# PacificBiosciences/ccs

Hardware: AMD Instinct MI355X
Metric: ZMWs/sec (HiFi reads/sec), 10-pass x 10 kb synthetic (higher is better)
Workload: dtype f32

## Files before the change

ccs_amd/csrc/ccsx_api.cpp:

```cpp
#include <hip/hip_runtime.h>

#include <algorithm>
#include <cmath>
#include <cstdio>
#include <cstdlib>
#include <cstring>
#include <mutex>
#include <string>
#include <vector>

#include "ccsx.h"
#include "ccsx_internal.h"
#include "ccsx_kernels.h"

#define HIPTRY(expr)                                                                                           \
    do {                                                                                                       \
        hipError_t e_ = (expr);                                                                                \
        if (e_ != hipSuccess) {                                                                                \
            ccsx_set_error(std::string(#expr) + ": " + hipGetErrorString(e_));                                 \
            return -2;                                                                                         \
        }                                                                                                      \
    } while (0)

#define CCSX_SLOTS 3
// ... 909 lines not shown
}
int ccsx_polish_batch(ccsx_handle h, const ccsx_batch *b, const ccsx_drafts *drafts, ccsx_results *res, uint32_t flags)
{
    ccsx_ticket t;
    if (int rc = ccsx_submit_polish(h, b, drafts, res, flags, &t)) return rc;
    return ccsx_wait(h, t);
}

static Slot *slot_of(ccsx_handle h, ccsx_ticket t)
{
    if (!h || t < 0) return nullptr;
    Slot &S = h->slot[t % CCSX_SLOTS];
    return S.ticket == t ? &S : nullptr;
}

int ccsx_wait(ccsx_handle h, ccsx_ticket ticket)
{
    Slot *S = slot_of(h, ticket);
    if (!S) { ccsx_set_error("ccsx_wait: unknown or recycled ticket"); return -1; }
    HIPTRY(hipSetDevice(h->device));
    return retire(h, *S);
}

int ccsx_poll(ccsx_handle h, ccsx_ticket ticket)
{
    Slot *S = slot_of(h, ticket);
    if (!S) { ccsx_set_error("ccsx_poll: unknown or recycled ticket"); return -1; }
    const hipError_t e = hipEventQuery(S->ev_done);
    if (e == hipErrorNotReady) return 0;
    if (e != hipSuccess) { ccsx_set_error(std::string("ccsx_poll: ") + hipGetErrorString(e)); return -2; }
    HIPTRY(hipSetDevice(h->device));
    return retire(h, *S) ? -2 : 1;
}

int ccsx_ticket_timings(ccsx_handle h, ccsx_ticket ticket, ccsx_timings *t)
{
    Slot *S = slot_of(h, ticket);
    if (!S || !t || !(S->ran || S->tm_ok)) { ccsx_set_error("ccsx_ticket_timings: unknown ticket"); return -1; }
    if (S->tm_ok) { *t = S->tm; return 0; }
    HIPTRY(hipSetDevice(h->device));
    return slot_timings(h, *S, t);
}

static int upload_impl(ccsx_handle h, const ccsx_batch *b, bool pile, bool tandem = false, int min_tandem = 0)
{
    if (!h) { ccsx_set_error("ccsx_upload: null handle"); return -1; }
    HIPTRY(hipSetDevice(h->device));
    for (auto &S : h->slot) if (int rc = retire(h, S)) return rc;
    Slot &S = h->slot[0];
    S.ticket = -1;
    const int rc = stage(h, S, b, h->s_comp, pile, tandem, min_tandem);
    if (rc) { S.staged = false; return rc; }
    S.mode = CCSX_RUN_FUSED;
    HIPTRY(hipStreamSynchronize(h->s_comp));
    h->last = 0;
    return 0;
}

int ccsx_upload(ccsx_handle h, const ccsx_batch *b) { return upload_impl(h, b, false); }

int ccsx_run(ccsx_handle h)
{
    if (!h || !h->slot[0].staged || h->slot[0].mode != CCSX_RUN_FUSED) { ccsx_set_error("ccsx_run: no batch uploaded for the fused path: call ccsx_upload first"); return -1; }
    HIPTRY(hipSetDevice(h->device));
    h->last = 0;
    return launch(h, h->slot[0]);
}

int ccsx_sync(ccsx_handle h)
{
    if (!h) return -1;
    HIPTRY(hipSetDevice(h->device));
    HIPTRY(hipStreamSynchronize(h->s_draft));
    HIPTRY(hipStreamSynchronize(h->s_comp));
    Slot &S = h->slot[h->last];
#ifdef CCSX_PROFILE_PHASES
    if (S.staged && S.ran) {
        unsigned long long ph[16];
        HIPTRY(hipMemcpy(ph, S.P.phase, sizeof(ph), hipMemcpyDeviceToHost));
        static const char *nm[8] = {"prologue", "tables+lanes", "chunk plan", "fill", "score", "select/apply", "qv+store", "validity+list"};
        unsigned long long tot = 0;
        for (int i = 0; i < 8; ++i) tot += ph[i];
        for (int i = 0; i < 8; ++i) std::fprintf(stderr, "[ccsx phase] %-14s %6.2f %%  (%llu cycles)\n", nm[i], tot ? 100.0 * ph[i] / tot : 0.0, ph[i]);
        static const char *pn[6] = {"thr setup+read", "thr traceback", "thr ids+zero", "thr records", "thr order", "thr col records"};
        unsigned long long pt = 0;
        for (int i = 8; i < 14; ++i) pt += ph[i];
        for (int i = 8; i < 14; ++i) std::fprintf(stderr, "[ccsx phase] %-14s %6.2f %%  (%llu cycles)\n", pn[i - 8], pt ? 100.0 * ph[i] / pt : 0.0, ph[i]);
    }
#endif
#ifdef CCSX_DEBUG_CHECKS
    if (S.staged) {
        int32_t dbg[2] = {0, 0};
        HIPTRY(hipMemcpy(dbg, S.P.debug, 8, hipMemcpyDeviceToHost));
        if (dbg[0]) { ccsx_set_error("device bounds check failed: code " + std::to_string(dbg[0]) + " at kernel line " + std::to_string(dbg[1])); return -3; }
    }
#endif
    (void)S;
    return 0;
}

int ccsx_download(ccsx_handle h, ccsx_results *res)
{
    if (!h || !h->slot[0].ran || h->slot[0].mode != CCSX_RUN_FUSED || !res) { ccsx_set_error("ccsx_download: nothing to download: ccsx_upload + ccsx_run first"); return -1; }
    Slot &S = h->slot[0];
    if (int rc = check_results(S, res, S.P.out_kin != nullptr)) return rc;
    HIPTRY(hipSetDevice(h->device));
    if (int rc = enqueue_download(S, res, h->s_comp)) return rc;
    HIPTRY(hipStreamSynchronize(h->s_comp));
    finish_outputs(S, res, nullptr);
    return 0;
}

int ccsx_consensus_batch(ccsx_handle h, const ccsx_batch *b, ccsx_results *res)
{
    int rc;
    if ((rc = ccsx_upload(h, b))) return rc;
    if ((rc = ccsx_run(h))) return rc;
    if ((rc = ccsx_sync(h))) return rc;
    return ccsx_download(h, res);
}

int ccsx_pileup_rule_version(void) { return 1; }

int ccsx_consensus_pileup(ccsx_handle h, const ccsx_batch *b, ccsx_results *res, ccsx_pileup *pile)
{
    if (!h || !b || !res || !pile) { ccsx_set_error("ccsx_consensus_pileup: null argument"); return -1; }
    int rc;
    if ((rc = upload_impl(h, b, true))) return rc;
    Slot &S = h->slot[0];
    if ((rc = check_pile(S, pile))) return rc;
    if ((rc = ccsx_run(h)) || (rc = ccsx_sync(h)) || (rc = ccsx_download(h, res))) return rc;
    if ((rc = enqueue_pile_download(S, pile, h->s_comp))) return rc;
    HIPTRY(hipStreamSynchronize(h->s_comp));
    return 0;
}

int ccsx_tandem_rule_version(void) { return 1; }

int ccsx_consensus_extras(ccsx_handle h, const ccsx_batch *b, ccsx_results *res, const ccsx_extras *ex)
{
    if (!h || !b || !res) { ccsx_set_error("ccsx_consensus_extras: null argument"); return -1; }
    bool tandem = false;
    if (extras_want(ex, &tandem)) return -1;
    ccsx_pileup *pile = ex ? ex->pile : nullptr;
    int rc;
    if ((rc = upload_impl(h, b, pile != nullptr, tandem, tandem ? ex->min_tandem_repeat_length : 0))) return rc;
    Slot &S = h->slot[0];
    if (pile && (rc = check_pile(S, pile))) return rc;
    if ((rc = ccsx_run(h)) || (rc = ccsx_sync(h)) || (rc = ccsx_download(h, res))) return rc;
    if (pile && (rc = enqueue_pile_download(S, pile, h->s_comp))) return rc;
    if (tandem && ex->tandem_len) HIPTRY(hipMemcpyAsync(ex->tandem_len, S.P.tlen, (size_t)S.P.n_zmw * 4, hipMemcpyDeviceToHost, h->s_comp));
    HIPTRY(hipStreamSynchronize(h->s_comp));
    return 0;
}

int ccsx_consensus_hd(ccsx_handle h, const ccsx_batch *b, ccsx_results *res, const ccsx_extras *ex, const ccsx_hd_request *hd)
{
    ccsx_hd_opts hdo{};
    if (b && hd_request_check(hd, b, &hdo, "ccsx_consensus_hd")) return -1;
    if (!h || !b || !res || !hd) { ccsx_set_error("ccsx_consensus_hd: null argument"); return -1; }
    bool tandem = false;
    if (extras_want(ex, &tandem)) return -1;
    ccsx_pileup *pile = ex ? ex->pile : nullptr;
    int rc;
    if ((rc = upload_impl(h, b, pile != nullptr, tandem, tandem ? ex->min_tandem_repeat_length : 0))) return rc;
    Slot &S = h->slot[0];
    if (pile && (rc = check_pile(S, pile))) return rc;
    if ((rc = check_results(S, res, S.P.out_kin != nullptr))) return rc;
    if ((rc = hd_table(h)) || (rc = hd_attach(h, S, hdo, hd->split, h->s_comp))) return rc;
    HIPTRY(hipStreamSynchronize(h->s_comp));
// ... 228 lines not shown
```

ccs_amd/csrc/ccsx_kernels.hip:

```cpp
#include <hip/hip_runtime.h>
#include <stdint.h>
#include <cstdio>
#include <cstdlib>

#include "ccsx.h"
#include "ccsx_kernels.h"
#include "wave_ops.h"

#define LANDED(x) asm volatile("" : "+v"(x))

#if (defined(CCSX_EXP_NO_FILL) || defined(CCSX_EXP_NO_SCORE) || defined(CCSX_EXP_ONE_ROUND) || defined(CCSX_EXP_ALL_VALID) || defined(CCSX_EXP_CHEAP_VALIDITY) || \
     defined(CCSX_EXP_NO_ROWS) || defined(CCSX_EXP_NO_SCORE_LOG) || defined(CCSX_EXP_SKIP_ROUND2_SCORE) || defined(CCSX_EXP_NO_QV_EXP) || defined(CCSX_EXP_REPEAT) || defined(CCSX_EXP_NO_BANDMASK) || \
     defined(CCSX_EXP_HOT_PROLOGUE) || defined(CCSX_EXIT_AFTER_PROLOGUE)) && !defined(CCSX_EXPERIMENT)
#error "CCSX_EXP_* / CCSX_EXIT_AFTER_PROLOGUE switches produce wrong results: build them with -DCCSX_EXPERIMENT (never ship such a library)"
#endif
#define CCSX_STR2(x) #x
#define CCSX_STR(x) CCSX_STR2(x)
int ccsx_kernel_is_experiment()
{
#ifdef CCSX_EXPERIMENT
    return 1;
#else
    return 0;
#endif
// ... 669 lines not shown
        }
        if (multim) {
            const int np = (rec.x >> 8) & 15;
            const bool act = live && k < n0;
            for (int q = 1; q < CCSX_MAXPRED; ++q) {
                if ((actm & M_SGT(np, q)) == 0ull) break;
                const bool on = act && np > q;
                int pq = q == 1 ? rec.z : rec.w, plo = q == 1 ? plo1 : plo2;
                if (q >= 3) {
                    if (on) {
                        pq = pxw[(size_t)k * 4 + (q - 3)];
                        if (k - pq > PRING) plo = kinfo[pq].x; else plo = LDS_I32(kinBase + (uint32_t)(pq & (PRING - 1)) * 16);
                    }
                    LANDED(pq); LANDED(plo);
                }
                const bool farq = on && k - pq > PRING;
                const int off = r0w - plo;
                const int w = imed3(off + 3, 1, PGS - 3);
                const uint32_t src = ringBase + (on ? (uint32_t)(pq & (PRING - 1)) : (uint32_t)PRING) * (PGS * 4) + ((uint32_t)w << 2);
                int x0 = LDS_I32(src), y0 = LDS_I32(src + 4), y1 = LDS_I32(src + 8);
                if (__builtin_expect(M_NE0(farq ? 1 : 0) != 0ull, 0)) {
                    if (farq) {
                        const int32_t *Mu = Mcol + (size_t)pq * PB;
                        const int o = off - 1;
                        x0 = (unsigned)o < (unsigned)PB ? Mu[o] : NEGV;
                        y0 = (unsigned)(o + 1) < (unsigned)PB ? Mu[o + 1] : NEGV;
                        y1 = (unsigned)(o + 2) < (unsigned)PB ? Mu[o + 2] : NEGV;
                    }
                    LANDED(x0); LANDED(y0); LANDED(y1);
                }
                const int mq = q << 1;
                int c;
                c = x0 + s0;     if (on && c > b0) { b0 = c; m0 = mq; }
                c = y0 + SC_DEL; if (on && c > b0) { b0 = c; m0 = mq | 1; }
                c = y0 + s1;     if (on && c > b1) { b1 = c; m1 = mq; }
                c = y1 + SC_DEL; if (on && c > b1) { b1 = c; m1 = mq | 1; }
            }
        }
        { const int c = b0 + SC_INS; if (c > b1) { b1 = c; m1 = 15; } }
        {
            const int S = row_scan_max_i32(b1 + l8);
            const int Sp = __builtin_amdgcn_update_dpp(-(1 << 30), S, DPP_ROW_SHR(1), 0xf, 0xf, false);
            const int c0v = Sp - (l8 - 8 - SC_INS);
            const int c1v = Sp - (l8 - 8 - 2 * SC_INS);
            if (c0v > b0) { b0 = c0v; m0 = 15; }
            if (c1v > b1) { b1 = c1v; m1 = 15; }
        }
        if (r0w > I || b0 < NEGV / 2) b0 = NEGV;
        if (r0w >= I || b1 < NEGV / 2) b1 = NEGV;
        int cm, br;
        {
            const int f = -(1 << 24);
            const int k0_ = ((b0 > f ? b0 : f) * 64) | kRow0, k1_ = ((b1 > f ? b1 : f) * 64) | kRow1;
            const int key = row_allmax_i32(k0_ > k1_ ? k0_ : k1_);
            cm = key >> 6; br = (lo + 63) - (key & 63);
        }
        if (__builtin_expect((actm & M_SGT(lo + PB, I)) != 0ull, 0)) {
            const int e = r0w == I ? b0 : (r0w + 1 == I ? b1 : NEGV);
            const int ev = __builtin_amdgcn_ds_bpermute(bcastAddr, row_scan_max_i32(e));
            if (live && k < n0 && ev > NEGV / 2 && ev > bs) { bs = ev; kend = k; }
        }
        if (live && k < n0) {
            *(int2 *)&sRing[gq][k & (PRING - 1)][4 + l2] = make_int2(b0, b1);
            *mvp = (uint8_t)(m0 | (m1 << 4));
            if (l == 0) {
                sKin[gq][k & (PRING - 1)] = make_int4(lo, cm, br, 0);
                *lop = lo;
            }
            if (__builtin_expect((rec.x & CREC_NEED) != 0, 0)) {
                *(int2 *)Mp = make_int2(b0, b1);
                if (l == 0) *kip = make_int4(lo, cm, br, p0);
            }
        }
    }
#undef M_NE0
#undef M_SLT
#undef M_SGT
#undef M_UGT
#undef LDS_I32
    __threadfence_block();
    if (live && l == 0) { st[ST_KEND] = kend; st[ST_BS] = bs; }
}

__global__ __launch_bounds__(64) __attribute__((amdgpu_waves_per_eu(8, 8))) void k_poa_thread(KParams P, int z0, int pass, int rr, int b0)
{
    const int bx = (int)blockIdx.x + b0;
    __shared__ __attribute__((aligned(16))) uint8_t sMv[TB_BLOCK * POA_MV_BYTES];
    const int lane = threadIdx.x;
    uint32_t *sread = dyn_lds;
    PoaSlot g = poa_slot(P, bx);
    if (z0 + bx >= P.n_zmw) return;
    if (!g.st[ST_LIVE] || !g.st[ST_OK] || rr >= g.st[ST_NPOA]) return;
    TPH_T0();
    const int z = rfl(P.zmw_perm[z0 + bx]);
    const int r0 = rfl(P.read_off[z]);
    const int bb = rfl(g.st[ST_BB]), nreads = rfl(g.st[ST_NREADS]), npoa = rfl(g.st[ST_NPOA]);
    const int r = r0 + (bb + rr < nreads ? bb + rr : bb + rr - nreads);
    const uint8_t *rb = P.bases + P.base_off[r];
    const int I = rfl((int)(P.base_off[r + 1] - P.base_off[r]));
    const int kend = rfl(g.st[ST_KEND]), bsc = rfl(g.st[ST_BS]);
    if (kend < 0 || bsc < I) return;
    const int rev = rfl(((P.flags[r] & 1) != g.st[ST_REV0]) ? 1 : 0);
    const int vcap = rfl(P.vcap[z]);
    const int n0 = rfl(g.st[ST_N]);
    const int par = rfl(g.st[ST_PAR]);
    const int4 *crec = par ? g.crec1 : g.crec0, *pxc = par ? g.px1 : g.px0;
    int4 *crec_nx = par ? g.crec0 : g.crec1, *px_nx = par ? g.px0 : g.px1;
    load_read_packed(sread, rb, I, rev, lane);
    __syncthreads();
    TPH(8);
    {
        int k = kend, i = I;
        int4 kiN = make_int4(0, 0, 0, -1), crN = make_int4(0, -1, -1, -1);
        int kbN = -1;
        uint4 mvN0 = make_uint4(0, 0, 0, 0);
        auto fetch = [&](int kb_) {
            const int kk = kb_ + lane;
            kbN = kb_;
            kiN = make_int4(0, 0, 0, -1); crN = make_int4(0, -1, -1, -1);
            if (kb_ >= 0) {
                if (kk < n0) { crN = crec[kk]; kiN = make_int4(g.loK[kk], 0, 0, crN.y); }
                mvN0 = ((const uint4 *)(g.mvK + (size_t)kb_ * POA_MV_BYTES))[lane];
            }
        };
        fetch((k / TB_BLOCK) * TB_BLOCK);
        while (k >= 0) {
            const int kb = (k / TB_BLOCK) * TB_BLOCK;
            if (kbN != kb) fetch(kb);
            __syncthreads();
            const int4 kiL = kiN, crL = crN;
            const int metaL = crN.x;
            ((uint4 *)sMv)[lane] = mvN0;
            fetch(kb - TB_BLOCK);
            __syncthreads();
            while (k >= kb) {
                int kl = k - kb;
                int mknown;
                {
                    const int kls = kl - lane;
                    const int src = kls & 63;
                    const int lo_s = __shfl(kiL.x, src), pp_s = __shfl(kiL.w, src);
                    const int off = i - lane - lo_s;
                    const bool inb = kls >= 0 && i - lane >= 1 && (unsigned)off < (unsigned)PB;
                    const int m_s = inb ? ((sMv[kls * POA_MV_BYTES + (off >> 1)] >> ((off & 1) << 2)) & 15) : 255;
                    const unsigned long long simple = __ballot(m_s == 0 && pp_s == k - lane - 1);
                    const int R = (simple == ~0ull) ? 64 : __ffsll((long long)~simple) - 1;
                    if (R > 0) {
                        const int meta_s = __shfl(metaL, src);
                        if (lane < R) {
                            const int ir = i - lane - 1;
                            g.pathv[ir] = ((meta_s & 3) == read_base_packed(sread, ir)) ? k - lane : -1;
                        }
                        k -= R; i -= R;
                        if (R >= 64 || k < kb) continue;
                        kl = k - kb;
                    }
                    mknown = rl(m_s, R);
                }
                const int lo_k = rl(kiL.x, kl);
                CHK(i - lo_k >= 0 && i - lo_k < PB && i >= 0, 101);
                const int mo = i - lo_k;
                const int m = mknown != 255 ? mknown : rfl((sMv[kl * POA_MV_BYTES + (mo >> 1)] >> ((mo & 1) << 2)) & 15);
                const int t = m == 15 ? MV_INS : (m & 1), slot = m >> 1;
                CHK(i >= 1 || t == MV_DEL, 102);
                if (t == MV_INS) { if (lane == 0) g.pathv[i - 1] = -1; --i; continue; }
                const int meta = rl(metaL, kl);
                const int np = (meta >> 8) & 15;
                int up;
                if (np == 0) up = -1;
                else if (slot == 0) up = rl(kiL.w, kl);
                else if (slot == 1) up = rl(crL.z, kl);
                else if (slot == 2) up = rl(crL.w, kl);
                else up = rfl(((const int32_t *)pxc)[(size_t)k * 4 + (slot - 3)]);
                if (t == MV_DIAG) {
                    if (lane == 0) g.pathv[i - 1] = ((meta & 3) == read_base_packed(sread, i - 1)) ? k : -1;
                    --i;
                }
                CHK(up < k && up >= -1, 103);
                k = up;
            }
            k = rfl(k); i = rfl(i);
        }
        for (int q = lane; q < i; q += LANES) g.pathv[q] = -1;
    }
    __threadfence_block();
    TPH(9);
    int32_t *cnt = g.bestK;
    auto newpos = [&](int q) -> int { return q + cnt[q]; };
    for (int q = lane; q <= n0; q += LANES) { cnt[q] = 0; g.onpK[q] = 0; }
    __threadfence_block();
    TPH(10);
    int lastEx = -1, nnew = 0;
    for (int c0 = 0; c0 < I; c0 += 2 * LANES) {
        int w[2], wn[2], ex[2];
        bool valid[2], isnew[2], lastOfRun[2];
#pragma unroll
        for (int u = 0; u < 2; ++u) {
            const int i = c0 + u * LANES + lane;
            valid[u] = i < I;
            const int ic = valid[u] ? i : I - 1;
            w[u] = g.pathv[ic];
            wn[u] = g.pathv[ic + 1 < I ? ic + 1 : ic];
        }
#pragma unroll
        for (int u = 0; u < 2; ++u) {
            const int i = c0 + u * LANES + lane;
            isnew[u] = valid[u] && w[u] < 0;
            nnew += __popcll(__ballot(isnew[u]));
            const int incl = wave_scan_max_i32((valid[u] && !isnew[u]) ? i : -1);
            int e = wave_shr1_i32(incl, -1);
            e = e > lastEx ? e : lastEx;
            ex[u] = e;
            const int li = rl(incl, 63);
            lastEx = li > lastEx ? li : lastEx;
            lastOfRun[u] = isnew[u] && ((i + 1 >= I) || (wn[u] >= 0));
        }
        int av[2];
#pragma unroll
        for (int u = 0; u < 2; ++u) av[u] = g.pathv[(lastOfRun[u] && ex[u] >= 0) ? ex[u] : 0];
#pragma unroll
        for (int u = 0; u < 2; ++u) {
            const int i = c0 + u * LANES + lane;
            if (valid[u] && !isnew[u]) g.onpK[w[u]] = 1;
            if (lastOfRun[u]) {
                const int ap = ex[u] >= 0 ? av[u] : -1;
                CHK(ap >= -1 && ap < n0, 106);
                cnt[ap + 1] = i - ex[u];
            }
        }
    }
    nnew = rfl(nnew);
    if (n0 + nnew > vcap) { if (lane == 0) g.st[ST_OK] = 0; return; }
    __threadfence_block();
    TPH(11);
    int carry = 0;
    for (int c0 = 0; c0 <= n0; c0 += 4 * LANES) {
        int cv[4];
#pragma unroll
        for (int u = 0; u < 4; ++u) { const int q = c0 + u * LANES + lane; cv[u] = cnt[q <= n0 ? q : n0]; }
#pragma unroll
        for (int u = 0; u < 4; ++u) {
            const int q = c0 + u * LANES + lane;
            const int incl = wave_scan_add_i32(q <= n0 ? cv[u] : 0);
            if (q <= n0) cnt[q] = carry + incl;
            carry += rl(incl, 63);
        }
    }
    const int n = n0 + nnew;
    for (int q = lane; q < n; q += LANES) g.needK[q] = 0;
    __threadfence_block();
    auto carry_over = [&](int q, int kn, int4 rec, int4 &pxr) -> int4 {
        const int np = (rec.x >> 8) & 15;
        rec.x &= ~CREC_FAR0;
        if (np > 0) { rec.y = newpos(rec.y); if (kn - rec.y > PRING) { g.needK[rec.y] = 1; rec.x |= CREC_FAR0; } }
        if (np > 1) { rec.z = newpos(rec.z); if (kn - rec.z > PRING) g.needK[rec.z] = 1; }
        if (np > 2) { rec.w = newpos(rec.w); if (kn - rec.w > PRING) g.needK[rec.w] = 1; }
        if (np > 3) {
            pxr = pxc[q];
            for (int e = 3; e < np; ++e) { const int pn = newpos(int4_get(pxr, e - 3)); int4_set(pxr, e - 3, pn); if (kn - pn > PRING) g.needK[pn] = 1; }
        }
        return rec;
    };
    for (int q0 = 0; q0 < n0; q0 += 2 * LANES) {
        int4 rec[2]; int kn[2]; bool go[2];
#pragma unroll
        for (int u = 0; u < 2; ++u) {
            const int q = q0 + u * LANES + lane;
            go[u] = q < n0 && !g.onpK[q < n0 ? q : 0];
            rec[u] = make_int4(0, -1, -1, -1); kn[u] = 0;
            if (go[u]) { rec[u] = crec[q]; kn[u] = newpos(q); }
        }
#pragma unroll
        for (int u = 0; u < 2; ++u) if (go[u]) {
            const int q = q0 + u * LANES + lane;
            int4 pxr = make_int4(-1, -1, -1, -1);
            const int4 r = carry_over(q, kn[u], rec[u], pxr);
            CHK(kn[u] >= 0 && kn[u] < n, 105);
            crec_nx[kn[u]] = r;
            if (((r.x >> 8) & 15) > 3) px_nx[kn[u]] = pxr;
        }
    }
    TPH(12);
    lastEx = -1;
    int prevP = -1;
    for (int c0 = 0; c0 < I; c0 += LANES) {
        const int i = c0 + lane;
        const bool valid = i < I;
        const int w = g.pathv[valid ? i : I - 1];
        const bool isnew = valid && w < 0;
        const int incl = wave_scan_max_i32((valid && !isnew) ? i : -1);
        int ex = wave_shr1_i32(incl, -1);
        ex = ex > lastEx ? ex : lastEx;
        { const int li = rl(incl, 63); lastEx = li > lastEx ? li : lastEx; }
        const int av = g.pathv[(isnew && ex >= 0) ? ex : 0];
        int4 rec = make_int4(0, -1, -1, -1);
        if (valid && !isnew) rec = crec[w];
        const int qa = valid ? (isnew ? (ex >= 0 ? av : 0) : w) : 0;
        int P = newpos(qa);
        if (isnew) P = (ex >= 0 ? P + 1 : 0) + (i - ex - 1);
        if (!valid) P = -1;
        int Pp = wave_shr1_i32(P, prevP);
        prevP = rl(P, 63);
        if (valid) {
            CHK(P >= 0 && P < n, 104);
            int4 pxr = make_int4(-1, -1, -1, -1);
            bool pxdirty = false;
            if (isnew) rec = make_int4(read_base_packed(sread, i) | ((Pp >= 0 ? 1 : 0) << 8) | (1 << CREC_NREADS_SHIFT), Pp, -1, -1);
            else {
                rec = carry_over(w, P, rec, pxr);
                rec.x += 1 << CREC_NREADS_SHIFT;
                if (Pp >= 0) {
                    const int np = (rec.x >> 8) & 15;
                    bool found = false;
                    if (np > 0) found |= rec.y == Pp;
                    if (np > 1) found |= rec.z == Pp;
                    if (np > 2) found |= rec.w == Pp;
                    for (int e = 3; e < np; ++e) found |= int4_get(pxr, e - 3) == Pp;
                    if (!found && np < CCSX_MAXPRED) {
                        if (np == 0) rec.y = Pp; else if (np == 1) rec.z = Pp; else if (np == 2) rec.w = Pp; else { int4_set(pxr, np - 3, Pp); pxdirty = true; }
                        rec.x += 1 << 8;
                        if (P - Pp > PRING) { g.needK[Pp] = 1; if (np == 0) rec.x |= CREC_FAR0; }
                    }
                }
            }
            crec_nx[P] = rec;
            if (((rec.x >> 8) & 15) > 3 || pxdirty) px_nx[P] = pxr;
        }
    }
    __threadfence_block();
    if (lane == 0) { g.st[ST_N] = n; g.st[ST_NADDED] += 1; g.st[ST_PAR] ^= 1; }
    (void)npoa;
    TPH(13);
}

__global__ __launch_bounds__(64) __attribute__((amdgpu_waves_per_eu(8, 8))) void k_poa_finish(KParams P, int z0, int pass, int b0)
{
    const int bx = (int)blockIdx.x + b0;
    const int lane = threadIdx.x;
    PoaSlot g = poa_slot(P, bx);
    if (z0 + bx >= P.n_zmw) return;
    if (!g.st[ST_LIVE]) return;
    const int z = rfl(P.zmw_perm[z0 + bx]);
    const int ok = rfl(g.st[ST_OK]), n = rfl(g.st[ST_N]), nadded = rfl(g.st[ST_NADDED]);
    const int4 *crec = g.st[ST_PAR] ? g.crec1 : g.crec0;
    const int32_t *pxw = (const int32_t *)(g.st[ST_PAR] ? g.px1 : g.px0);
    int Ld = 0, nw = 0, stat = -1;
    if (ok && n > 0) {
        int kbest = -1, sb = NEGV, best_prev = 0;
        for (int kb = 0; kb < n; kb += LANES) {
            const int kkL = kb + lane;
            int4 cL = make_int4(0, -1, -1, -1);
            if (kkL < n) cL = crec[kkL];
            const int nblk = (n - kb) < LANES ? (n - kb) : LANES;
            const int npL = (cL.x >> 8) & 15;
            const int wL = kkL < n ? 2 * ((cL.x >> CREC_NREADS_SHIFT) & 127) - nadded : 0;
            const int Pw = wave_scan_add_i32(wL);
            const bool headL = kkL < n && (lane == 0 || npL != 1 || cL.y != kkL - 1);
            unsigned long long heads = __ballot(headL);
            const unsigned long long headmask = heads;
            int hb = 0, bpv = kkL - 1;
            while (heads) {
                const int j = (int)__ffsll((long long)heads) - 1;
                heads &= heads - 1;
                const int k = kb + j;
                const int np = rl(npL, j);
                int b = 0, p = -1;
                for (int q = 0; q < np; ++q) {
                    int pu;
                    if (q < 3) pu = q == 0 ? rl(cL.y, j) : (q == 1 ? rl(cL.z, j) : rl(cL.w, j));
                    else pu = rfl(pxw[(size_t)k * 4 + (q - 3)]);
                    CHK(pu >= 0 && pu < k, 108);
                    int bu;
                    if (pu >= kb) {
                        const int pj = pu - kb;
                        const int hd = 63 - __clzll((long long)(headmask & ((2ull << pj) - 1ull)));
                        bu = rl(hb, hd) + rl(Pw, pj) - rl(Pw, hd);
                    } else bu = pu == kb - 1 ? best_prev : rfl(g.bestK[pu]);
// ... 2689 lines not shown
            const int i = atomicAdd(&sV[5], 1);
            if (i < CAP) sBuf[i] = ((unsigned long long)end << 32) | ((unsigned long long)s << 24) | ((unsigned long long)dist << 16) | (unsigned long long)(end - start);
        });
        __syncthreads();
    }
    const int nk = min(sV[5], CAP), n_listed = min(n_hits, NH);
    for (int i = tid; i < nk; i += NT) {
        const unsigned long long key = sBuf[i];
        int rank = 0;
        for (int q = 0; q < nk && rank < NH; ++q) rank += sBuf[q] < key ? 1 : 0;
        if (rank < NH) {
            const int end = (int)(key >> 32);
            list[rank * 3] = end - (int)(key & 0xffffu); list[rank * 3 + 1] = end; list[rank * 3 + 2] = (int)((key >> 24) & 0xffu) | ((int)((key >> 16) & 0xffu) << 8);
        }
    }
    if (tid < NH && tid >= n_listed) { list[tid * 3] = 0; list[tid * 3 + 1] = 0; list[tid * 3 + 2] = 0; }
    int cov = 0;
    for (int w = tid; w < words; w += NT) cov += __popc(sUnion[w]);
    if (cov) atomicAdd(&sV[4], cov);
    {
        const int seg = (L + NT - 1) / NT, a = min(tid * seg, L), b = min(a + seg, L);
        int lead = -1, run = 0, inner = 0;
        for (int i = a; i < b; ++i) {
            if ((sUnion[i >> 5] >> (i & 31)) & 1u) { if (lead < 0) lead = run; inner = max(inner, run); run = 0; }
            else ++run;
        }
        sSeg[tid][0] = lead < 0 ? b - a : lead; sSeg[tid][1] = run; sSeg[tid][2] = lead < 0 ? -1 : inner;
    }
    __syncthreads();
    if (tid == 0) {
        int run = 0, gap = 0;
        for (int t = 0; t < NT; ++t) {
            if (sSeg[t][2] < 0) { run += sSeg[t][0]; continue; }
            gap = max(gap, max(run + sSeg[t][0], sSeg[t][2]));
            run = sSeg[t][1];
        }
        gap = max(gap, run);
        const ccsx_adapter_opts &o = P.adapt;
        const int first = n_hits ? sV[1] : -1, last = sV[2];
        int v = 0;
        if (n_hits >= o.min_copies && gap <= o.max_insert) v |= CCSX_ADAPTER_CONCAT;
        if (n_hits >= 1 && (first <= o.end_slack || last >= L - o.end_slack)) v |= CCSX_ADAPTER_NEAR_END;
        out[0] = 1; out[n] = v; out[2 * n] = n_hits; out[3 * n] = n_listed; out[4 * n] = sV[4]; out[5 * n] = gap; out[6 * n] = first; out[7 * n] = last;
        out[8 * n] = sV[3];
    }
}

#define LAUNCH_CHECK(name) do { if (hipGetLastError() != hipSuccess && !failed) failed = name; } while (0)
#define CALL_CHECK(fn, ...) do { if (fn(__VA_ARGS__) != hipSuccess && !failed) failed = #fn; } while (0)
const char *ccsx_launch_all(const KParams &P, hipStream_t st, hipStream_t st_polish, hipEvent_t *ev , int mode, hipStream_t st_aux, hipEvent_t *ev_aux )
{
    const char *failed = nullptr;
    if (ev) CALL_CHECK(hipEventRecord, ev[0], st);
    CALL_CHECK(hipMemsetAsync, P.ticket_poa, 0, 256, st);
    CALL_CHECK(hipMemsetAsync, P.avalid, 0, (size_t)(P.n_reads > 0 ? P.n_reads : 1), st);
    if (P.tflag) { CALL_CHECK(hipMemsetAsync, P.tflag, 0, (size_t)P.n_zmw * 4, st); CALL_CHECK(hipMemsetAsync, P.tlen, 0, (size_t)P.n_zmw * 4, st); }
    {
        int n = P.n_zmw * CCSX_NCTX;
        hipLaunchKernelGGL(k_setup, dim3((n + 255) / 256), dim3(256), 0, st, P);
        LAUNCH_CHECK("k_setup");
    }
    trace_sync(st, "k_setup");
    if (ev) CALL_CHECK(hipEventRecord, ev[1], st);
    const size_t lds_read = (((size_t)P.maxL_max + 15) / 16) * 4 + 64 + 4 * (CCSX_MAX_PASSES + 1);
    const bool caller_drafts = mode == CCSX_RUN_POLISH || mode == CCSX_RUN_HD;
    if (caller_drafts) {
        hipLaunchKernelGGL(k_draft_in, dim3(P.n_zmw), dim3(64), 0, st, P);
        LAUNCH_CHECK("k_draft_in");
    }
    for (int pass = 0; pass < ((P.opts.no_fallback_draft || caller_drafts) ? 1 : 3); ++pass) {
        int cov = pass ? 2 * P.opts.max_poa_cov : P.opts.max_poa_cov;
        if (cov > PW_MAXREADS_SPEC) cov = PW_MAXREADS_SPEC;
        if (cov > P.max_reads) cov = P.max_reads;
        for (int z0 = 0; z0 < P.n_zmw && !caller_drafts; z0 += P.poa_slots) {
            const int nb = (P.n_zmw - z0) < P.poa_slots ? (P.n_zmw - z0) : P.poa_slots;
            auto poa_range = [&](hipStream_t s, int g0, int ng, hipEvent_t after_first_dp, hipEvent_t before_first_dp) {
                hipLaunchKernelGGL(k_poa_init, dim3(ng), dim3(64), lds_read, s, P, z0, pass, g0);
                LAUNCH_CHECK("k_poa_init");
                if (before_first_dp) CALL_CHECK(hipStreamWaitEvent, s, before_first_dp, 0);
                for (int rr = 1; rr < cov && pass < 2; ++rr) {
                    hipLaunchKernelGGL(k_poa_dp, dim3((ng + 3) / 4), dim3(64), 0, s, P, z0, pass, rr, g0 / 4);
                    LAUNCH_CHECK("k_poa_dp");
                    if (rr == 1 && after_first_dp) CALL_CHECK(hipEventRecord, after_first_dp, s);
                    hipLaunchKernelGGL(k_poa_thread, dim3(ng), dim3(64), lds_read, s, P, z0, pass, rr, g0);
                    LAUNCH_CHECK("k_poa_thread");
                }
                if (pass < 2) {
                    hipLaunchKernelGGL(k_poa_finish, dim3(ng), dim3(64), 0, s, P, z0, pass, g0);
                    LAUNCH_CHECK("k_poa_finish");
                }
            };
            if (st_aux && ev_aux && pass == 0 && cov > 1 && nb >= 4096) {
                const int ha = ((nb / 2) + 3) & ~3;
                CALL_CHECK(hipEventRecord, ev_aux[0], st);
                CALL_CHECK(hipStreamWaitEvent, st_aux, ev_aux[0], 0);
                poa_range(st, 0, ha, ev_aux[1], nullptr);
                poa_range(st_aux, ha, nb - ha, nullptr, ev_aux[1]);
                CALL_CHECK(hipEventRecord, ev_aux[2], st_aux);
                CALL_CHECK(hipStreamWaitEvent, st, ev_aux[2], 0);
            } else poa_range(st, 0, nb, nullptr, nullptr);
        }
        trace_sync(st, "k_poa");
        if (P.tflag) {
            hipLaunchKernelGGL(k_sdust, dim3(P.n_zmw), dim3(64), (size_t)CCSX_SDUST_TABLE_BYTES + (size_t)P.sdust_words * 4, st, P, pass);
            LAUNCH_CHECK("k_sdust");
        }
        if (ev && pass == 0) CALL_CHECK(hipEventRecord, ev[2], st);
        CALL_CHECK(hipMemsetAsync, P.align_retry, 0, 64, st);
        bool tb_aside_out = false; int tb_launches = 0;
        {
            const size_t lds16 = 4 * (CH16 / 16 + 3) * sizeof(uint32_t);
            static const bool aside_ok = [] { const char *e = getenv("CCSX_TB_ASIDE"); return !(e && e[0] == '0'); }();
            const bool aside = aside_ok && st_aux && ev_aux && pass == 0 && P.n_quads >= 4096;
            bool tb_aside = false;
            int c = 0;
            for (int qb = 0; qb < P.n_quads; qb += P.align16_slots, ++c) {
                const int nb = (P.n_quads - qb) < P.align16_slots ? (P.n_quads - qb) : P.align16_slots;
                const int region = P.align16_regions > 1 ? (c & 1) : 0;
                if (aside && c >= 2) CALL_CHECK(hipStreamWaitEvent, st, ev_aux[5 + (c & 1)], 0);
                if (aside && c >= 1 && P.align16_regions <= 1) CALL_CHECK(hipStreamWaitEvent, st, ev_aux[5 + ((c - 1) & 1)], 0);
                hipLaunchKernelGGL(k_align16, dim3(nb), dim3(64), lds16, st, P, qb, pass, region);
                LAUNCH_CHECK("k_align16");
                hipStream_t s_tb = st;
                if (aside) {
                    CALL_CHECK(hipEventRecord, ev_aux[3 + (c & 1)], st);
                    CALL_CHECK(hipStreamWaitEvent, st_aux, ev_aux[3 + (c & 1)], 0);
                    s_tb = st_aux; tb_aside = true;
                }
                hipLaunchKernelGGL(k_align16_tb, dim3((4 * nb + 63) / 64), dim3(64), 0, s_tb, P, qb, nb, region);
                LAUNCH_CHECK("k_align16_tb");
                if (aside) CALL_CHECK(hipEventRecord, ev_aux[5 + (c & 1)], st_aux);
            }
            tb_launches = c;
            tb_aside_out = tb_aside;
        }
        {
            const int g = P.align_slots < 1 ? 1 : (P.align_slots > 4096 ? 4096 : P.align_slots);
            hipLaunchKernelGGL(k_align, dim3(g), dim3(64), lds_read, st, P, pass);
            LAUNCH_CHECK("k_align");
        }
        trace_sync(st, "k_align");
        if (P.align_slots >= 2) {
            const int g = P.align_slots / 2 > 2048 ? 2048 : P.align_slots / 2;
            hipLaunchKernelGGL(k_rescue, dim3(g), dim3(64), lds_read, st, P, pass);
            LAUNCH_CHECK("k_rescue");
        }
        if (tb_aside_out) for (int c = tb_launches > 2 ? tb_launches - 2 : 0; c < tb_launches; ++c)
            CALL_CHECK(hipStreamWaitEvent, st, ev_aux[5 + (c & 1)], 0);
        hipLaunchKernelGGL(k_post, dim3((P.n_zmw + 255) / 256), dim3(256), 0, st, P, pass);
        LAUNCH_CHECK("k_post");
    }
    if (mode == CCSX_RUN_DRAFT) {
        if (ev) for (int k : {3, 6, 4, 5}) CALL_CHECK(hipEventRecord, ev[k], st);
        return failed;
    }
    hipLaunchKernelGGL(k_wmap, dim3(1), dim3(1024), 0, st, P);
    LAUNCH_CHECK("k_wmap");
    hipLaunchKernelGGL(k_wmap_fill, dim3((P.n_zmw + 3) / 4), dim3(256), 0, st, P);
    LAUNCH_CHECK("k_wmap_fill");
    if (mode == CCSX_RUN_FUSED && P.fold_zi) {
        hipLaunchKernelGGL(k_fold, dim3(P.n_zmw), dim3(CCSX_FOLD_THREADS), (size_t)P.fold_bins * 4, st, P);
        LAUNCH_CHECK("k_fold");
        trace_sync(st, "k_fold");
    }
    if (mode == CCSX_RUN_FUSED && P.adapt_zi) {
        hipLaunchKernelGGL(k_adapter, dim3(P.n_zmw), dim3(CCSX_ADAPTER_THREADS), (size_t)P.adapt_words * 8, st, P);
// ... 68 lines not shown
```

Measured before the change: 38470.

## Split POA traceback into a separate kernel packing four ZMWs per wave

Moves the POA traceback out of k_poa_thread into a new k_poa_tb kernel. Each 64-lane wave runs four ZMWs in 16-lane groups, using wave-level barriers, prefetched global loads done with inline assembly, and ballot/bpermute run skipping. Read-base matching is deferred: pathv stores the node position tagged with the node's base, and consumers decode it with path_pos against the read base. The goal is to stop a single ZMW's serial traceback from holding a whole wave, at the cost of an extra kernel launch per read and a more complex path encoding.

```diff
diff --git a/ccs_amd/csrc/ccsx_api.cpp b/ccs_amd/csrc/ccsx_api.cpp
--- a/ccs_amd/csrc/ccsx_api.cpp
+++ b/ccs_amd/csrc/ccsx_api.cpp
@@ -1015,10 +1015,11 @@
         unsigned long long tot = 0;
         for (int i = 0; i < 8; ++i) tot += ph[i];
         for (int i = 0; i < 8; ++i) std::fprintf(stderr, "[ccsx phase] %-14s %6.2f %%  (%llu cycles)\n", nm[i], tot ? 100.0 * ph[i] / tot : 0.0, ph[i]);
-        static const char *pn[6] = {"thr setup+read", "thr traceback", "thr ids+zero", "thr records", "thr order", "thr col records"};
+        static const char *pn[6] = {"thr setup+read", "thr (unused)", "thr ids+zero", "thr records", "thr order", "thr col records"};
         unsigned long long pt = 0;
         for (int i = 8; i < 14; ++i) pt += ph[i];
         for (int i = 8; i < 14; ++i) std::fprintf(stderr, "[ccsx phase] %-14s %6.2f %%  (%llu cycles)\n", pn[i - 8], pt ? 100.0 * ph[i] / pt : 0.0, ph[i]);
+        std::fprintf(stderr, "[ccsx phase] %-14s %llu cycles\n[ccsx phase] %-14s %llu cycles  (k_poa_thread, all phases: %llu)\n", "tb setup", ph[14], "tb walk", ph[15], pt);
     }
 #endif
 #ifdef CCSX_DEBUG_CHECKS
diff --git a/ccs_amd/csrc/ccsx_kernels.hip b/ccs_amd/csrc/ccsx_kernels.hip
--- a/ccs_amd/csrc/ccsx_kernels.hip
+++ b/ccs_amd/csrc/ccsx_kernels.hip
@@ -775,10 +775,121 @@
     if (live && l == 0) { st[ST_KEND] = kend; st[ST_BS] = bs; }
 }
 
+#define TB_PATH_BASE_SHIFT 28
+#define TB_PATH_POS ((1 << TB_PATH_BASE_SHIFT) - 1)
+__device__ __forceinline__ int path_pos(int w, int read_base) { return (w >= 0 && (w >> TB_PATH_BASE_SHIFT) == read_base) ? (w & TB_PATH_POS) : -1; }
+
+__global__ __launch_bounds__(64) void k_poa_tb(KParams P, int z0, int pass, int rr, int b0)
+{
+    const int bx = (int)blockIdx.x + b0;
+    __shared__ __attribute__((aligned(16))) uint8_t sMv[4][TB_BLOCK * POA_MV_BYTES];
+    __shared__ __attribute__((aligned(16))) int4 sCr[4][TB_BLOCK];
+    const int lane = threadIdx.x, h = lane >> 4, l = lane & 15;
+    const int zi = z0 + 4 * bx + h;
+    const bool have = zi < P.n_zmw && 4 * bx + h < P.poa_slots;
+    const PoaSlot g = poa_slot(P, have ? 4 * bx + h : 4 * bx);
+    bool live = have && g.st[ST_LIVE] && g.st[ST_OK] && rr < g.st[ST_NPOA];
+    int I = 0, kend = -1, n0 = 1, par = 0;
+    if (live) {
+        const int z = P.zmw_perm[zi];
+        const int r0 = P.read_off[z];
+        const int bb = g.st[ST_BB], nreads = g.st[ST_NREADS];
+        const int r = r0 + (bb + rr < nreads ? bb + rr : bb + rr - nreads);
+        I = (int)(P.base_off[r + 1] - P.base_off[r]);
+        kend = g.st[ST_KEND];
+        n0 = g.st[ST_N]; par = g.st[ST_PAR];
+        live = kend >= 0 && g.st[ST_BS] >= I;
+    }
+    if (!__any(live)) return;
+    TPH_T0();
+    const int4 *crec = par ? g.crec1 : g.crec0;
+    const int32_t *pxw = (const int32_t *)(par ? g.px1 : g.px0);
+    const int32_t *loK = g.loK;
+    const uint4 *mvK = (const uint4 *)g.mvK;
+    int32_t *pathv = g.pathv;
+    static_assert(POA_MV_BYTES == 16 && TB_BLOCK == 64, "k_poa_tb: a move row is one uint4, a block is four columns per lane");
+    int k = live ? kend : -1, i = I;
+    int kb = -1, kbN = -1;
+    typedef int tb_v4i __attribute__((ext_vector_type(4)));
+#define TB_LOAD128(dst, ptr) asm volatile("global_load_dwordx4 %0, %1, off" : "+v"(dst) : "v"(ptr) : "memory")
+#define TB_LOAD32(dst, ptr) asm volatile("global_load_dword %0, %1, off" : "+v"(dst) : "v"(ptr) : "memory")
+    tb_v4i crN[4], mvN[4]; int loN[4];
+#pragma unroll
+    for (int j = 0; j < 4; ++j) { crN[j] = (tb_v4i){0, -1, -1, -1}; loN[j] = 0; mvN[j] = (tb_v4i){0, 0, 0, 0}; }
+    auto fetch = [&](int kb_) {
+        kbN = kb_;
+        if (kb_ >= 0) {
+#pragma unroll
+            for (int j = 0; j < 4; ++j) {
+                const int kk = kb_ + 16 * j + l, kc = kk < n0 ? kk : n0 - 1;
+                const int4 *pc = crec + kc; const int32_t *pl = loK + kc; const uint4 *pm = mvK + kk;
+                TB_LOAD128(crN[j], pc); TB_LOAD32(loN[j], pl); TB_LOAD128(mvN[j], pm);
+            }
+        }
+    };
+    if (live) fetch(k & ~(TB_BLOCK - 1));
+    TPH(14);
+    for (;;) {
+        const bool act = k >= 0;
+        if (!__any(act)) break;
+        const int kbw = k & ~(TB_BLOCK - 1);
+        if (__any(act && kbw != kb)) {
+            if (act && kbw != kb) {
+                if (kbN != kbw) fetch(kbw);
+                asm volatile("s_waitcnt vmcnt(0)"
+                             : "+v"(crN[0]), "+v"(crN[1]), "+v"(crN[2]), "+v"(crN[3]), "+v"(mvN[0]), "+v"(mvN[1]), "+v"(mvN[2]), "+v"(mvN[3]),
+                               "+v"(loN[0]), "+v"(loN[1]), "+v"(loN[2]), "+v"(loN[3]) : : "memory");
+#pragma unroll
+                for (int j = 0; j < 4; ++j) {
+                    const int c = 16 * j + l;
+                    sCr[h][c] = make_int4((crN[j].x & 3) | (((crN[j].x >> 8) & 15) << 2) | (loN[j] << 8), crN[j].y, crN[j].z, crN[j].w);
+                    ((tb_v4i *)sMv[h])[c] = mvN[j];
+                }
+                kb = kbw;
+                fetch(kb - TB_BLOCK);
+            }
+            __builtin_amdgcn_fence(__ATOMIC_RELEASE, "wavefront");
+            __builtin_amdgcn_wave_barrier();
+            __builtin_amdgcn_fence(__ATOMIC_ACQUIRE, "wavefront");
+        }
+        const int kls = k - kb - l;
+        const bool cv = act && kls >= 0;
+        const int cc = cv ? kls : 0;
+        const int4 cr = sCr[h][cc];
+        const int row = i - l;
+        const int off = row - (int)((unsigned)cr.x >> 8);
+        const bool inb = cv && row >= 0 && (unsigned)off < (unsigned)PB;
+        const int oc = inb ? off : 0;
+        const int m = inb ? ((sMv[h][cc * POA_MV_BYTES + (oc >> 1)] >> ((oc & 1) << 2)) & 15) : 255;
+        const unsigned long long sm = __ballot(m == 0 && row >= 1 && cr.y == k - l - 1);
+        const unsigned f = (unsigned)(sm >> (h << 4)) & 0xffffu;
+        const int R = __ffs((int)(~f | 0x10000u)) - 1;
+        const int k1 = k - R, i1 = i - R;
+        const bool stopv = act && R < 16 && k1 >= kb;
+        const bool mine = stopv && l == R;
+        const bool ins = m == 15, del = !ins && (m & 1);
+        const int slot = m >> 1, np = (cr.x >> 2) & 15;
+        int up = np == 0 ? -1 : (slot == 0 ? cr.y : (slot == 1 ? cr.z : cr.w));
+        const bool needpx = mine && m < 14 && np > 0 && slot >= 3;
+        if (__builtin_expect(__any(needpx), 0)) { if (needpx) up = pxw[(size_t)k1 * 4 + (slot - 3)]; LANDED(up); }
+        const bool bad = m == 255 || (!del && row < 1) || (!ins && up >= k1);
+        int nk = ins ? k1 : up, ni = del ? i1 : i1 - 1;
+        if (bad) { nk = -1; ni = i1; }
+        if (l < R || (mine && !del && !bad)) pathv[row - 1] = (mine && ins) ? -1 : ((k - l) | ((cr.x & 3) << TB_PATH_BASE_SHIFT));
+        const int src = ((lane & 48) | (R & 15)) << 2;
+        const int bk = __builtin_amdgcn_ds_bpermute(src, nk), bi = __builtin_amdgcn_ds_bpermute(src, ni);
+        k = stopv ? bk : k1;
+        i = stopv ? bi : i1;
+    }
+    if (live) for (int q = l; q < i; q += 16) pathv[q] = -1;
+    TPH(15);
+#undef TB_LOAD128
+#undef TB_LOAD32
+}
+
 __global__ __launch_bounds__(64) __attribute__((amdgpu_waves_per_eu(8, 8))) void k_poa_thread(KParams P, int z0, int pass, int rr, int b0)
 {
     const int bx = (int)blockIdx.x + b0;
-    __shared__ __attribute__((aligned(16))) uint8_t sMv[TB_BLOCK * POA_MV_BYTES];
     const int lane = threadIdx.x;
     uint32_t *sread = dyn_lds;
     PoaSlot g = poa_slot(P, bx);
@@ -802,80 +913,6 @@
     load_read_packed(sread, rb, I, rev, lane);
     __syncthreads();
     TPH(8);
-    {
-        int k = kend, i = I;
-        int4 kiN = make_int4(0, 0, 0, -1), crN = make_int4(0, -1, -1, -1);
-        int kbN = -1;
-        uint4 mvN0 = make_uint4(0, 0, 0, 0);
-        auto fetch = [&](int kb_) {
-            const int kk = kb_ + lane;
-            kbN = kb_;
-            kiN = make_int4(0, 0, 0, -1); crN = make_int4(0, -1, -1, -1);
-            if (kb_ >= 0) {
-                if (kk < n0) { crN = crec[kk]; kiN = make_int4(g.loK[kk], 0, 0, crN.y); }
-                mvN0 = ((const uint4 *)(g.mvK + (size_t)kb_ * POA_MV_BYTES))[lane];
-            }
-        };
-        fetch((k / TB_BLOCK) * TB_BLOCK);
-        while (k >= 0) {
-            const int kb = (k / TB_BLOCK) * TB_BLOCK;
-            if (kbN != kb) fetch(kb);
-            __syncthreads();
-            const int4 kiL = kiN, crL = crN;
-            const int metaL = crN.x;
-            ((uint4 *)sMv)[lane] = mvN0;
-            fetch(kb - TB_BLOCK);
-            __syncthreads();
-            while (k >= kb) {
-                int kl = k - kb;
-                int mknown;
-                {
-                    const int kls = kl - lane;
-                    const int src = kls & 63;
-                    const int lo_s = __shfl(kiL.x, src), pp_s = __shfl(kiL.w, src);
-                    const int off = i - lane - lo_s;
-                    const bool inb = kls >= 0 && i - lane >= 1 && (unsigned)off < (unsigned)PB;
-                    const int m_s = inb ? ((sMv[kls * POA_MV_BYTES + (off >> 1)] >> ((off & 1) << 2)) & 15) : 255;
-                    const unsigned long long simple = __ballot(m_s == 0 && pp_s == k - lane - 1);
-                    const int R = (simple == ~0ull) ? 64 : __ffsll((long long)~simple) - 1;
-                    if (R > 0) {
-                        const int meta_s = __shfl(metaL, src);
-                        if (lane < R) {
-                            const int ir = i - lane - 1;
-                            g.pathv[ir] = ((meta_s & 3) == read_base_packed(sread, ir)) ? k - lane : -1;
-                        }
-                        k -= R; i -= R;
-                        if (R >= 64 || k < kb) continue;
-                        kl = k - kb;
-                    }
-                    mknown = rl(m_s, R);
-                }
-                const int lo_k = rl(kiL.x, kl);
-                CHK(i - lo_k >= 0 && i - lo_k < PB && i >= 0, 101);
-                const int mo = i - lo_k;
-                const int m = mknown != 255 ? mknown : rfl((sMv[kl * POA_MV_BYTES + (mo >> 1)] >> ((mo & 1) << 2)) & 15);
-                const int t = m == 15 ? MV_INS : (m & 1), slot = m >> 1;
-                CHK(i >= 1 || t == MV_DEL, 102);
-                if (t == MV_INS) { if (lane == 0) g.pathv[i - 1] = -1; --i; continue; }
-                const int meta = rl(metaL, kl);
-                const int np = (meta >> 8) & 15;
-                int up;
-                if (np == 0) up = -1;
-                else if (slot == 0) up = rl(kiL.w, kl);
-                else if (slot == 1) up = rl(crL.z, kl);
-                else if (slot == 2) up = rl(crL.w, kl);
-                else up = rfl(((const int32_t *)pxc)[(size_t)k * 4 + (slot - 3)]);
-                if (t == MV_DIAG) {
-                    if (lane == 0) g.pathv[i - 1] = ((meta & 3) == read_base_packed(sread, i - 1)) ? k : -1;
-                    --i;
-                }
-                CHK(up < k && up >= -1, 103);
-                k = up;
-            }
-            k = rfl(k); i = rfl(i);
-        }
-        for (int q = lane; q < i; q += LANES) g.pathv[q] = -1;
-    }
     __threadfence_block();
     TPH(9);
     int32_t *cnt = g.bestK;
@@ -892,8 +929,9 @@
             const int i = c0 + u * LANES + lane;
             valid[u] = i < I;
             const int ic = valid[u] ? i : I - 1;
-            w[u] = g.pathv[ic];
-            wn[u] = g.pathv[ic + 1 < I ? ic + 1 : ic];
+            const int in_ = ic + 1 < I ? ic + 1 : ic;
+            w[u] = path_pos(g.pathv[ic], read_base_packed(sread, ic));
+            wn[u] = path_pos(g.pathv[in_], read_base_packed(sread, in_));
         }
 #pragma unroll
         for (int u = 0; u < 2; ++u) {
@@ -910,7 +948,7 @@
         }
         int av[2];
 #pragma unroll
-        for (int u = 0; u < 2; ++u) av[u] = g.pathv[(lastOfRun[u] && ex[u] >= 0) ? ex[u] : 0];
+        for (int u = 0; u < 2; ++u) av[u] = g.pathv[(lastOfRun[u] && ex[u] >= 0) ? ex[u] : 0] & TB_PATH_POS;
 #pragma unroll
         for (int u = 0; u < 2; ++u) {
             const int i = c0 + u * LANES + lane;
@@ -979,13 +1017,14 @@
     for (int c0 = 0; c0 < I; c0 += LANES) {
         const int i = c0 + lane;
         const bool valid = i < I;
-        const int w = g.pathv[valid ? i : I - 1];
+        const int ic = valid ? i : I - 1;
+        const int w = path_pos(g.pathv[ic], read_base_packed(sread, ic));
         const bool isnew = valid && w < 0;
         const int incl = wave_scan_max_i32((valid && !isnew) ? i : -1);
         int ex = wave_shr1_i32(incl, -1);
         ex = ex > lastEx ? ex : lastEx;
         { const int li = rl(incl, 63); lastEx = li > lastEx ? li : lastEx; }
-        const int av = g.pathv[(isnew && ex >= 0) ? ex : 0];
+        const int av = g.pathv[(isnew && ex >= 0) ? ex : 0] & TB_PATH_POS;
         int4 rec = make_int4(0, -1, -1, -1);
         if (valid && !isnew) rec = crec[w];
         const int qa = valid ? (isnew ? (ex >= 0 ? av : 0) : w) : 0;
@@ -3841,6 +3880,8 @@
                     hipLaunchKernelGGL(k_poa_dp, dim3((ng + 3) / 4), dim3(64), 0, s, P, z0, pass, rr, g0 / 4);
                     LAUNCH_CHECK("k_poa_dp");
                     if (rr == 1 && after_first_dp) CALL_CHECK(hipEventRecord, after_first_dp, s);
+                    hipLaunchKernelGGL(k_poa_tb, dim3((ng + 3) / 4), dim3(64), 0, s, P, z0, pass, rr, g0 / 4);
+                    LAUNCH_CHECK("k_poa_tb");
                     hipLaunchKernelGGL(k_poa_thread, dim3(ng), dim3(64), lds_read, s, P, z0, pass, rr, g0);
                     LAUNCH_CHECK("k_poa_thread");
                 }
```

New measurement: 38400. No clear change (-0.2%).
